# megvii-research/basedet

Hardware: AMD Instinct MI355X
Metric: images/sec training RetinaNet-R50-FPN 1333x800 (higher is better)
Workload: dtype bf16; 1 GPU; retinanet_r50_800x1344 train step (fwd+bwd+allreduce+SGD), DummyLoader boxes, random-init weights, inputs resident in HBM; per_gpu_batch=16, global_batch=16, parallelism=dp1

## Files before the change

### basedet_amd/_lib.py

```python
import ctypes as C
import os

import torch

_HERE = os.path.dirname(os.path.abspath(__file__))
LIB_PATH = os.environ.get("BASEDET_HIP_LIB") or os.path.join(_HERE, "lib", "libbasedet_hip.so")

BD_MAX_SEGS = 8
ABI_VERSION = 112
EPI_RELU, EPI_ADD_BEFORE, EPI_ADD_AFTER, EPI_MASK, EPI_SPARSE = 1, 2, 4, 8, 16


class BasedetHipError(RuntimeError):
    pass


class ConvDesc(C.Structure):
    _fields_ = [
        ("N", C.c_int32), ("Cin", C.c_int32), ("Cout", C.c_int32), ("R", C.c_int32), ("S", C.c_int32),
        ("stride", C.c_int32), ("pad", C.c_int32), ("nseg", C.c_int32),
        ("Hi", C.c_int32 * BD_MAX_SEGS), ("Wi", C.c_int32 * BD_MAX_SEGS),
        ("Ho", C.c_int32 * BD_MAX_SEGS), ("Wo", C.c_int32 * BD_MAX_SEGS),
        ("in_off", C.c_int32 * BD_MAX_SEGS), ("out_off", C.c_int32 * BD_MAX_SEGS),
        ("in_pix_per_img", C.c_int32), ("out_pix_per_img", C.c_int32),
        ("route", C.c_int32 * 4), ("sr_seed", C.c_uint32),
        ("gskip", C.c_int32), ("gskip_ws", C.c_void_p), ("gskip_ws_bytes", C.c_size_t),
        ("gskip_gmap", C.c_void_p), ("gskip_gmap_bytes", C.c_size_t), ("gskip_dxmap", C.c_void_p), ("gskip_dxmap_bytes", C.c_size_t),
        ("gskip_dx_clean", C.c_int32),
        ("fwd_map", C.c_void_p), ("fwd_map_bytes", C.c_size_t), ("fwd_clean", C.c_int32),
    ]


class PackDesc(C.Structure):
    _fields_ = [("w", C.c_void_p), ("row_scale", C.c_void_p), ("w_fwd", C.c_void_p), ("w_dgrad", C.c_void_p),
                ("Cout", C.c_int32), ("RS", C.c_int32), ("Cin", C.c_int32), ("block_start", C.c_int32)]


class ImageDesc(C.Structure):
    _fields_ = [("offset", C.c_int64), ("src_h", C.c_int32), ("src_w", C.c_int32), ("dst_h", C.c_int32), ("dst_w", C.c_int32),
                ("flip", C.c_int32), ("reserved_", C.c_int32 * 1)]


_P, _I, _L, _F, _Z = C.c_void_p, C.c_int, C.c_int64, C.c_float, C.c_size_t
_D = C.POINTER(ConvDesc)

SIGNATURES = {
    "bd_last_error_string": (C.c_char_p, []),
    "bd_version": (_I, []),
    "bd_conv_last_kernel": (C.c_char_p, []),
# ... 113 lines not shown
    "bd_rcnn_loss_fwd_bwd": (_I, [_P, _I, _I, _I, _P, _P, _I, _F, _P, _P, _P, _P]),
    "bd_det_scores": (_I, [_P, _I, _P, _I, _I, _L, _I, _P, _P]),
    "bd_det_select_workspace_bytes": (_Z, [_I, _I, _L, _I, _I]),
    "bd_det_select": (_I, [_P, _I, _P, _I, _I, _I, _L, _I, _I, _P, _P, _I, _F, _P, _P, _P, _P, _Z, _P]),
    "bd_rcnn_predict": (_I, [_P, _I, _I, _I, _P, _P, _I, _I, _P, _P, _P, _P, _P]),
    "bd_det_candidates": (_I, [_I, _P, _P, _P, _I, _I, _I, _P, _I, _P, _P, _L, _I, _I, _P, _P, _P, _L, _P, _P, _P, _P]),
    "bd_det_finalize": (_I, [_P, _P, _P, _P, _P, _I, _I, _I, _P, _I, _P, _P, _P, _P]),
    "bd_sgd_momentum_step": (_I, [_P, _P, _P, _L, _F, _F, _F, _F, _P]),
    "bd_ema_update": (_I, [_P, _P, _L, _F, _F, _P]),
    "bd_sgd_momentum_ema_step": (_I, [_P, _P, _P, _P, _L, _F, _F, _F, _F, _F, _F, _P]),
    "bd_swap_f32": (_I, [_P, _P, _L, _P]),
    "bd_adam_step": (_I, [_P, _P, _P, _P, _L] + [_F] * 10 + [_I, _P]),
    "bd_adam_ema_step": (_I, [_P, _P, _P, _P, _P, _L] + [_F] * 10 + [_I, _F, _F, _P]),
    "bd_sgd_nesterov_step": (_I, [_P, _P, _P, _L, _F, _F, _F, _F, _P]),
    "bd_sgd_nesterov_ema_step": (_I, [_P, _P, _P, _P, _L, _F, _F, _F, _F, _F, _F, _P]),
    "bd_clip_grad_value": (_I, [_P, _L, _F, _F, _F, _P]),
    "bd_clip_grad_norm_workspace_bytes": (_Z, []),
    "bd_clip_grad_norm": (_I, [_P, _L, _F, _F, _F, _P, _P, _Z, _P]),
    "bd_quantize_fp8": (_I, [_P, _L, _F, _P, _P]),
    "bd_weight_pack_fp8": (_I, [_P, _P, _I, _I, _I, _F, _P, _P, _P]),
    "bd_conv2d_fwd_fp8": (_I, [_D, _P, _P, _P, _P, _P, _P, _I, _P]),
    "bd_conv2d_fwd_fp8_ex": (_I, [_D, _P, _P, _P, _P, _P, _P, _P, _F, _I, _P]),
    "bd_quantize_bf8": (_I, [_P, _L, _F, _P, C.c_uint32, _P]),
    "bd_absmax_bf16": (_I, [_P, _L, _P, _P]),
    "bd_weight_pack_fp8_t": (_I, [_P, _P, _I, _I, _I, _F, _P, _P, _P]),
    "bd_conv2d_dgrad_fp8": (_I, [_D, _P, _P, _P, _P, _P, _P, _P, _F, _I, _P]),
    "bd_conv2d_wgrad_fp8_workspace_bytes": (_Z, [_D]),
    "bd_conv2d_wgrad_fp8": (_I, [_D, _P, _P, _F, _P, _P, _I, _P, _Z, _P]),
    "bd_conv1x1_fp8": (_I, [_D, _I, _P, _P, _P, _P, _P, _P, _P, _P, _P, _P, _F, _I, _P]),
    "bd_sigmoid_focal_loss_elem": (_I, [_P, _P, _L, _F, _F, _P, _P, _P, _P]),
# ... 75 lines not shown
```

### basedet_amd/build.py

```python
import hashlib
import os
import subprocess
import sys

HERE = os.path.dirname(os.path.abspath(__file__))
CSRC = os.path.join(HERE, "csrc")
OUT_DIR = os.path.join(HERE, "lib")
LIB = os.path.join(OUT_DIR, os.environ.get("BD_LIB_NAME", "libbasedet_hip.so"))
HIPCC = os.environ.get("HIPCC", "/opt/rocm/bin/hipcc")
ARCH = "gfx950"

SOURCES = {
    "image_ops.hip": [],
    "image_resize.hip": ["-ffp-contract=off"],
    "ema.hip": [],
    "optim.hip": ["-ffp-contract=off", "-fhip-fp32-correctly-rounded-divide-sqrt"],
    "h2d.hip": [],
    "conv_igemm.hip": [],
    "conv3x3.hip": [],
    "conv3x3_pp.hip": [],
    "gskip.hip": [],
    "conv3x3_pp128.hip": [],
    "conv1x1.hip": [],
    "conv1x1_ring.hip": [],
    "conv1x1_thin.hip": [],
    "bottleneck_fused.hip": [],
    "conv_fp8.hip": [],
    "conv3x3_pp8.hip": [],
    "conv_wgrad.hip": [],
    "conv_wgrad3x3.hip": [],
    "conv_wgrad3x3_ring.hip": [],
# ... 88 lines not shown
```

### basedet_amd/csrc/ema.hip

```cpp
#include "common.h"

namespace {

__global__ void ema_kernel(float* __restrict__ e, const float* __restrict__ w, long long n, float m, float one_minus_m) {
    for (long long i = (long long)blockIdx.x * blockDim.x + threadIdx.x; i * 4 < n; i += (long long)gridDim.x * blockDim.x) {
        const long long o = i * 4;
        if (o + 4 <= n) {
            f32x4_t ev = *reinterpret_cast<f32x4_t*>(e + o);
            const f32x4_t wv = *reinterpret_cast<const f32x4_t*>(w + o);
#pragma unroll
            for (int k = 0; k < 4; ++k) ev[k] = ema_elem(ev[k], wv[k], m, one_minus_m);
            *reinterpret_cast<f32x4_t*>(e + o) = ev;
        } else {
            for (long long k = o; k < n; ++k) e[k] = ema_elem(e[k], w[k], m, one_minus_m);
        }
    }
}

__global__ void sgd_ema_kernel(float* __restrict__ w, float* __restrict__ v, const float* __restrict__ g, float* __restrict__ e,
                               long long n, float lr, float momentum, float wd, float grad_scale, float m, float one_minus_m) {
    for (long long i = (long long)blockIdx.x * blockDim.x + threadIdx.x; i * 4 < n; i += (long long)gridDim.x * blockDim.x) {
        const long long o = i * 4;
        if (o + 4 <= n) {
            f32x4_t wv = *reinterpret_cast<f32x4_t*>(w + o);
            f32x4_t vv = *reinterpret_cast<f32x4_t*>(v + o);
            const f32x4_t gv = *reinterpret_cast<const f32x4_t*>(g + o);
            f32x4_t ev = *reinterpret_cast<f32x4_t*>(e + o);
#pragma unroll
            for (int k = 0; k < 4; ++k) {
                const float gg = gv[k] * grad_scale + wd * wv[k];
                vv[k] = momentum * vv[k] + gg;
                wv[k] -= lr * vv[k];
                ev[k] = ema_elem(ev[k], wv[k], m, one_minus_m);
            }
            *reinterpret_cast<f32x4_t*>(w + o) = wv;
            *reinterpret_cast<f32x4_t*>(v + o) = vv;
            *reinterpret_cast<f32x4_t*>(e + o) = ev;
        } else {
            for (long long k = o; k < n; ++k) {
                const float gg = g[k] * grad_scale + wd * w[k];
                v[k] = momentum * v[k] + gg;
                w[k] -= lr * v[k];
                e[k] = ema_elem(e[k], w[k], m, one_minus_m);
            }
        }
    }
}

__global__ void swap_kernel(float* __restrict__ a, float* __restrict__ b, long long n) {
    for (long long i = (long long)blockIdx.x * blockDim.x + threadIdx.x; i * 4 < n; i += (long long)gridDim.x * blockDim.x) {
        const long long o = i * 4;
        if (o + 4 <= n) {
            const f32x4_t av = *reinterpret_cast<const f32x4_t*>(a + o);
            const f32x4_t bv = *reinterpret_cast<const f32x4_t*>(b + o);
            *reinterpret_cast<f32x4_t*>(a + o) = bv;
            *reinterpret_cast<f32x4_t*>(b + o) = av;
        } else {
            for (long long k = o; k < n; ++k) {
// ... 48 lines not shown
```

### basedet_amd/csrc/image_ops.hip

```cpp
#include <stdarg.h>

#include <cmath>
#include "common.h"

static thread_local std::string g_bd_error = "";
int bd_num_cus() {
    static std::mutex mu;
    static int cached[256] = {0};
    int dev = 0;
    if (hipGetDevice(&dev) != hipSuccess || dev < 0 || dev > 255) return 256;
    std::lock_guard<std::mutex> g(mu);
    if (!cached[dev]) {
        int n = 0;
        cached[dev] = (hipDeviceGetAttribute(&n, hipDeviceAttributeMultiprocessorCount, dev) == hipSuccess && n > 0) ? n : 256;
    }
    return cached[dev];
}

void bd_set_error(const char* fmt, ...) {
    char buf[512];
    va_list ap;
    va_start(ap, fmt);
    vsnprintf(buf, sizeof(buf), fmt, ap);
    va_end(ap);
    g_bd_error = buf;
}
extern "C" const char* bd_last_error_string(void) { return g_bd_error.c_str(); }
static thread_local const char* g_bd_last_kernel = "";
void bd_note_kernel(const char* name) { g_bd_last_kernel = name; }
extern "C" const char* bd_conv_last_kernel(void) { return g_bd_last_kernel; }
extern "C" int bd_version(void) { return 112; }

namespace {

constexpr int HALO_Y = 3, HALO_X = 4;

__global__ void pad_normalize_kernel(const float* __restrict__ in, int N, int H, int W, int Hp, int Wp,
                                     float m0, float m1, float m2, float s0, float s1, float s2,
                                     bf16_raw* __restrict__ out) {
    const int Hb = Hp + 2 * HALO_Y, Wb = Wp + 2 * HALO_X;
    const long long total = (long long)N * Hb * Wb;
    for (long long i = (long long)blockIdx.x * blockDim.x + threadIdx.x; i < total; i += (long long)gridDim.x * blockDim.x) {
        const int xb = (int)(i % Wb);
        const long long t = i / Wb;
        const int yb = (int)(t % Hb);
        const int n = (int)(t / Hb);
// ... 295 lines not shown
        for (int k = 0; k < 32; ++k) t += red[k * 8 + cl];
        out[c] = accumulate ? out[c] + t : t;
    }
}

__global__ void sgd_kernel(float* __restrict__ w, float* __restrict__ v, const float* __restrict__ g, long long n,
                           float lr, float momentum, float wd, float grad_scale) {
    for (long long i = (long long)blockIdx.x * blockDim.x + threadIdx.x; i * 4 < n; i += (long long)gridDim.x * blockDim.x) {
        const long long e = i * 4;
        if (e + 4 <= n) {
            f32x4_t wv = *reinterpret_cast<f32x4_t*>(w + e);
            f32x4_t vv = *reinterpret_cast<f32x4_t*>(v + e);
            const f32x4_t gv = *reinterpret_cast<const f32x4_t*>(g + e);
#pragma unroll
            for (int k = 0; k < 4; ++k) {
                const float gg = gv[k] * grad_scale + wd * wv[k];
                vv[k] = momentum * vv[k] + gg;
                wv[k] -= lr * vv[k];
            }
            *reinterpret_cast<f32x4_t*>(w + e) = wv;
            *reinterpret_cast<f32x4_t*>(v + e) = vv;
        } else {
            for (long long k = e; k < n; ++k) {
                const float gg = g[k] * grad_scale + wd * w[k];
                v[k] = momentum * v[k] + gg;
                w[k] -= lr * v[k];
            }
        }
    }
}

}

extern "C" int bd_pad_normalize(const float* in, int N, int H, int W, int Hp, int Wp, const float* mean3,
                                const float* std3, void* out, bd_stream_t stream) {
    BD_REQUIRE(in && out && mean3 && std3, "pad_normalize: null pointer");
    BD_REQUIRE(Hp >= H && Wp >= W && N > 0, "pad_normalize: padded size smaller than input");
    const long long total = (long long)N * (Hp + 6) * (Wp + 8);
    hipLaunchKernelGGL(pad_normalize_kernel, dim3(grid_for(total)), dim3(256), 0, (hipStream_t)stream, in, N, H, W, Hp, Wp,
                       mean3[0], mean3[1], mean3[2], std3[0], std3[1], std3[2], (bf16_raw*)out);
    BD_CHECK_LAUNCH("bd_pad_normalize");
// ... 238 lines not shown
```

### basedet_amd/csrc/optim.hip

```cpp
#include "common.h"

namespace {

struct AdamArgs {
    float lr, beta1, one_minus_beta1, beta2, one_minus_beta2, bc1, bc2, eps, wd, grad_scale, ema_m, one_minus_ema_m;
};

template <bool DECOUPLED, bool EMA>
__device__ __forceinline__ void adam_elem(float& w, float& m, float& v, float g, float& e, const AdamArgs& a) {
    float gg = g * a.grad_scale;
    if (!DECOUPLED) gg = gg + a.wd * w;
    m = a.beta1 * m + a.one_minus_beta1 * gg;
    v = a.beta2 * v + a.one_minus_beta2 * (gg * gg);
    float d = (m / a.bc1) / (sqrtf(v / a.bc2) + a.eps);
    if (DECOUPLED) d = d + a.wd * w;
    w = w - a.lr * d;
    if (EMA) e = ema_elem(e, w, a.ema_m, a.one_minus_ema_m);
}

template <bool DECOUPLED, bool EMA>
__global__ void adam_kernel(float* __restrict__ w, float* __restrict__ m, float* __restrict__ v, const float* __restrict__ g,
                            float* __restrict__ e, long long n, AdamArgs a) {
    for (long long i = (long long)blockIdx.x * blockDim.x + threadIdx.x; i * 4 < n; i += (long long)gridDim.x * blockDim.x) {
        const long long o = i * 4;
        if (o + 4 <= n) {
            f32x4_t wv = *reinterpret_cast<f32x4_t*>(w + o);
            f32x4_t mv = *reinterpret_cast<f32x4_t*>(m + o);
            f32x4_t vv = *reinterpret_cast<f32x4_t*>(v + o);
            const f32x4_t gv = *reinterpret_cast<const f32x4_t*>(g + o);
            f32x4_t ev = {0.f, 0.f, 0.f, 0.f};
            if (EMA) ev = *reinterpret_cast<f32x4_t*>(e + o);
#pragma unroll
            for (int k = 0; k < 4; ++k) {
// ... 2 lines not shown
                wv[k] = wk; mv[k] = mk; vv[k] = vk; ev[k] = ek;
            }
            *reinterpret_cast<f32x4_t*>(w + o) = wv;
            *reinterpret_cast<f32x4_t*>(m + o) = mv;
            *reinterpret_cast<f32x4_t*>(v + o) = vv;
            if (EMA) *reinterpret_cast<f32x4_t*>(e + o) = ev;
        } else {
            for (long long k = o; k < n; ++k) {
                float wk = w[k], mk = m[k], vk = v[k], ek = EMA ? e[k] : 0.f;
                adam_elem<DECOUPLED, EMA>(wk, mk, vk, g[k], ek, a);
                w[k] = wk; m[k] = mk; v[k] = vk;
                if (EMA) e[k] = ek;
            }
        }
    }
}

template <bool EMA>
__device__ __forceinline__ void nesterov_elem(float& w, float& v, float g, float& e, float lr, float momentum, float wd, float grad_scale,
                                              float ema_m, float one_minus_ema_m) {
    const float gg = g * grad_scale + wd * w;
    v = momentum * v + gg;
    w -= lr * (gg + momentum * v);
    if (EMA) e = ema_elem(e, w, ema_m, one_minus_ema_m);
}

template <bool EMA>
__global__ void sgd_nesterov_kernel(float* __restrict__ w, float* __restrict__ v, const float* __restrict__ g, float* __restrict__ e,
                                    long long n, float lr, float momentum, float wd, float grad_scale, float ema_m,
                                    float one_minus_ema_m) {
    for (long long i = (long long)blockIdx.x * blockDim.x + threadIdx.x; i * 4 < n; i += (long long)gridDim.x * blockDim.x) {
        const long long o = i * 4;
        if (o + 4 <= n) {
            f32x4_t wv = *reinterpret_cast<f32x4_t*>(w + o);
            f32x4_t vv = *reinterpret_cast<f32x4_t*>(v + o);
            const f32x4_t gv = *reinterpret_cast<const f32x4_t*>(g + o);
            f32x4_t ev = {0.f, 0.f, 0.f, 0.f};
            if (EMA) ev = *reinterpret_cast<f32x4_t*>(e + o);
#pragma unroll
// ... 94 lines not shown
```

### basedet_amd/models/fpn_base.py

```python
import math

import numpy as np
import torch

from .. import ops
from ..data.raw import RawImageBatch
from ..ops import Geom
from ..streams import SideStreams, fork, join
from . import params as P
from .. import comm as _comm
from .engine import ConvLayer, DeconvLayer, FCLayer, ParamArena, TrainableStem
from .fp8_scaling import Fp8GradScaler, initial_grad_scale
from .live_norm import BatchNormState, LiveNorms
from .plan_arena import PlanArena, _Carver, _Plan, _round_up
from .wgrad_sched import WgradScheduler


class VecParam:

    def __init__(self, name, numel):
        self.name, self.numel = name, numel
        self.w = self.g = None

    def reserve(self, arena):
# ... 252 lines not shown
    def _q8_buf(self, key, nbytes):
        t = self._q8.get(key)
        if t is None or t.numel() < nbytes:
            t = self._q8[key] = torch.empty((int(nbytes),), dtype=torch.uint8, device=self.device)
        return t

    def load_weights(self, weights, strict=False):
        from ..utils.checkpoint import load_matched_weights
        return load_matched_weights(self, weights, strict)

    def repack_weights(self):
        ops.stem_weight_pack(self.stem_w, self.stem_scale, self.stem_packed)
        for c in self.convs.values():
            c.pack()

    def repack_trainable(self):
        self.fp8_scaler.apply_staged()
        if self._pack_table is None:
            ent = [(c.w, c.row_scale, c.w_fwd, c.w_dgrad, c.cout, c.k * c.k, c.cin) for c in self.convs.values()
                   if c.trainable and not isinstance(c, DeconvLayer)]
            self._pack_table = ops.build_pack_table(ent, self.device)
        ops.weight_pack_multi(self._pack_table)
        if self.stem is not None:
            ops.stem_weight_pack(self.stem_w, self.stem_scale, self.stem_packed)
        for c in self.upsample.values():
            c.pack()
        for c in self.convs.values():
            if (c.fp8 or c.fp8_1x1 or c.fp8_1x1_dgrad) and c.trainable:
                c.pack_fp8()
        if self.norms and not self.training:
            self._fold_norms()

    def _fold_norms(self, pack=True):
        if not self.norms:
            return
        for c in self.convs.values():
            if c.norm is None:
# ... 689 lines not shown
```

### basedet_amd/ops.py

```python
import ctypes as C
from dataclasses import dataclass, field
from typing import List, Optional

import torch

from . import _lib
from ._lib import ConvDesc, EPI_ADD_AFTER, EPI_ADD_BEFORE, EPI_MASK, EPI_RELU, EPI_SPARSE, check, f32arr, i32arr, ptr, stream_ptr


@dataclass
class Geom:
    N: int
    H: List[int]
    W: List[int]
    off: List[int] = field(default_factory=list)
    pix_per_img: int = 0

    def __post_init__(self):
        if not self.off:
            o = 0
            self.off = []
            for h, w in zip(self.H, self.W):
                self.off.append(o)
                o += h * w
# ... 295 lines not shown
        arr[i].w = w.data_ptr()
        arr[i].row_scale = rs.data_ptr() if rs is not None else None
        arr[i].w_fwd = wf.data_ptr() if wf is not None else None
        arr[i].w_dgrad = wd.data_ptr() if wd is not None else None
        arr[i].Cout, arr[i].RS, arr[i].Cin, arr[i].block_start = co, r, ci, start
        start += int(L().bd_weight_pack_blocks(co, r, ci))
    raw = np.frombuffer(bytes(arr), dtype=np.uint8).copy()
    return torch.from_numpy(raw).to(device), len(entries), start


def weight_pack_multi(table):
    t, n, blocks = table
    check(L().bd_weight_pack_multi(ptr(t), n, blocks, stream_ptr()), "bd_weight_pack_multi")


def colsum_workspace_bytes(Cn):
    return int(L().bd_colsum_workspace_bytes(Cn))


def colsum_bf16(g, rows, Cn, out, ws, accumulate=False, geom=None):
    if geom is None:
        n, ppi, off, cnt = 1, rows, 0, rows
    else:
        assert geom.nlev == 1
        n, ppi, off, cnt = geom.N, geom.pix_per_img, geom.off[0], geom.H[0] * geom.W[0]
    check(L().bd_colsum_bf16(ptr(g), n, ppi, off, cnt, Cn, ptr(out), int(accumulate), ptr(ws), ws.numel() * ws.element_size(),
                             stream_ptr()), "bd_colsum_bf16")
    return out


# ... 446 lines not shown
                                  stream_ptr()), "bd_fcos_offsets_fwd")
    return out


def fcos_offsets_workspace_bytes():
    return int(L().bd_fcos_offsets_workspace_bytes())


def fcos_offsets_bwd(raw, ld, scales, geom: Geom, strides, d_off, d_ctr, d_raw, dscale, ws):
    off, cnt = _lvl_arrays(geom)
    check(L().bd_fcos_offsets_bwd(ptr(raw), ld, ptr(scales), geom.N, geom.nlev, off, cnt, i32arr(strides), geom.pix_per_img, ptr(d_off),
                                  ptr(d_ctr), ptr(d_raw), ptr(dscale), ptr(ws), ws.numel() * ws.element_size(), stream_ptr()),
          "bd_fcos_offsets_bwd")


def sgd_momentum_step(w, v, g, lr, momentum, wd, grad_scale=1.0):
    check(L().bd_sgd_momentum_step(ptr(w), ptr(v), ptr(g), w.numel(), float(lr), float(momentum), float(wd),
                                   float(grad_scale), stream_ptr()), "bd_sgd_momentum_step")


def ema_coeffs(m):
    return float(m), float(1 - m)


def _same_f32(*ts):
    assert all(t.dtype == torch.float32 and t.numel() == ts[0].numel() for t in ts), "fp32 buffers of one length expected"


def ema_update(e, w, m):
    _same_f32(e, w)
    mm, om = ema_coeffs(m)
    check(L().bd_ema_update(ptr(e), ptr(w), e.numel(), mm, om, stream_ptr()), "bd_ema_update")


def sgd_momentum_ema_step(w, v, g, e, lr, momentum, wd, grad_scale, m):
    _same_f32(w, v, g, e)
    mm, om = ema_coeffs(m)
    check(L().bd_sgd_momentum_ema_step(ptr(w), ptr(v), ptr(g), ptr(e), w.numel(), float(lr), float(momentum), float(wd),
                                       float(grad_scale), mm, om, stream_ptr()), "bd_sgd_momentum_ema_step")


def swap_f32(a, b):
    _same_f32(a, b)
    check(L().bd_swap_f32(ptr(a), ptr(b), a.numel(), stream_ptr()), "bd_swap_f32")


def adam_coeffs(betas, step):
    b1, b2 = float(betas[0]), float(betas[1])
    return b1, 1 - b1, b2, 1 - b2, 1 - b1 ** step, 1 - b2 ** step


def adam_step(w, m, v, g, lr, betas, eps, wd, step, grad_scale=1.0, decoupled=False):
    _same_f32(w, m, v, g)
    check(L().bd_adam_step(ptr(w), ptr(m), ptr(v), ptr(g), w.numel(), float(lr), *adam_coeffs(betas, step), float(eps), float(wd),
                           float(grad_scale), int(bool(decoupled)), stream_ptr()), "bd_adam_step")


def adam_ema_step(w, m, v, g, e, lr, betas, eps, wd, step, grad_scale, decoupled, ema_m):
    _same_f32(w, m, v, g, e)
    mm, om = ema_coeffs(ema_m)
    check(L().bd_adam_ema_step(ptr(w), ptr(m), ptr(v), ptr(g), ptr(e), w.numel(), float(lr), *adam_coeffs(betas, step), float(eps),
                               float(wd), float(grad_scale), int(bool(decoupled)), mm, om, stream_ptr()), "bd_adam_ema_step")


def sgd_nesterov_step(w, v, g, lr, momentum, wd, grad_scale=1.0):
    _same_f32(w, v, g)
    check(L().bd_sgd_nesterov_step(ptr(w), ptr(v), ptr(g), w.numel(), float(lr), float(momentum), float(wd), float(grad_scale),
                                   stream_ptr()), "bd_sgd_nesterov_step")


def sgd_nesterov_ema_step(w, v, g, e, lr, momentum, wd, grad_scale, m):
    _same_f32(w, v, g, e)
    mm, om = ema_coeffs(m)
    check(L().bd_sgd_nesterov_ema_step(ptr(w), ptr(v), ptr(g), ptr(e), w.numel(), float(lr), float(momentum), float(wd),
                                       float(grad_scale), mm, om, stream_ptr()), "bd_sgd_nesterov_ema_step")


class WgradQueue:

    def __init__(self):
        self._h = C.c_void_p()
        check(L().bd_wgrad_queue_create(C.byref(self._h)), "bd_wgrad_queue_create")

    def wgrad(self, d, x, g, dw, dbias, ws, row_scale=None, accumulate=False):
        check(L().bd_conv2d_wgrad_queued(self._h, C.byref(_stamp(d)), ptr(x), ptr(g), ptr(row_scale), ptr(dw), ptr(dbias), int(accumulate), ptr(ws),
                                         ws.numel() * ws.element_size(), stream_ptr()), "bd_conv2d_wgrad_queued")
# ... 79 lines not shown
```

### basedet_amd/solver/__init__.py

```python
import torch

from .. import comm as _comm
from .. import ops
from ..streams import fork, join
from ..utils.registry import registers


class _ParamGroupView(dict):
    pass


def _moments_out(model, buf):
    w = model.arena.w
    ops.swap_f32(buf, w)
    try:
        states = model.state_dict()
    finally:
        ops.swap_f32(buf, w)
    return {k: states[k] for k in model.state_dict_trainable_names()}


def _moments_in(model, buf, values):
    own = model.state_dict()
    trainable = set(model.state_dict_trainable_names())
    missing = sorted(trainable - set(values))
    if missing:
        raise ValueError(f"optimizer state lacks {len(missing)} trainable parameter(s), e.g. {missing[0]!r}")
    merged = {k: (values[k] if k in trainable else v) for k, v in own.items()}
    w = model.arena.w
    try:
        ops.swap_f32(buf, w)
        try:
            model._bind_params(merged)
        finally:
            ops.swap_f32(buf, w)
    finally:
        model.repack_weights()


class SGD:

    def __init__(self, model, lr, weight_decay, momentum=0.9, nesterov=False):
        if nesterov and momentum <= 0:
            raise ValueError("SGD: nesterov=True requires a momentum > 0")
        self.model = model
        self.nesterov = bool(nesterov)
        self.step_count = 0
        self.param_groups = [_ParamGroupView(lr=lr, weight_decay=weight_decay, momentum=momentum)]

    def step(self, grad_scale=1.0, ema=None):
        a = self.model.arena
        g = self.param_groups[0]
        m = ema.fused_momentum() if ema is not None else None
        plain, fused = (ops.sgd_nesterov_step, ops.sgd_nesterov_ema_step) if self.nesterov else \
            (ops.sgd_momentum_step, ops.sgd_momentum_ema_step)
        if m is None:
            plain(a.w, a.v, a.g, g["lr"], g["momentum"], g["weight_decay"], grad_scale)
        else:
            fused(a.w, a.v, a.g, ema.e, g["lr"], g["momentum"], g["weight_decay"], grad_scale, m)
        self.step_count += 1
        self.model.repack_trainable()
        return self

    def clear_grad(self):
        return self

    def state_dict(self):
        return {"step": self.step_count, "momentum_buffer": _moments_out(self.model, self.model.arena.v)}

    def load_state_dict(self, states):
        self.step_count = int(states["step"])
        _moments_in(self.model, self.model.arena.v, states["momentum_buffer"])


class Adam:

    decoupled = False

    def __init__(self, model, lr, weight_decay, betas=(0.9, 0.999), eps=1e-8):
        if len(betas) != 2 or not all(0.0 <= float(b) < 1.0 for b in betas):
            raise ValueError(f"{type(self).__name__}: betas must be two values in [0, 1), got {betas!r}")
        betas = (float(betas[0]), float(betas[1]))
        if eps < 0:
            raise ValueError(f"{type(self).__name__}: eps must not be negative, got {eps!r}")
        self.model = model
        self.step_count = 0
        self.param_groups = [_ParamGroupView(lr=lr, weight_decay=weight_decay, betas=betas, eps=eps)]
        a = model.arena
        self.exp_avg_sq = torch.zeros(a.total, dtype=torch.float32, device=a.w.device)

    def step(self, grad_scale=1.0, ema=None):
        a = self.model.arena
        g = self.param_groups[0]
        m = ema.fused_momentum() if ema is not None else None
        t = self.step_count + 1
        if m is None:
            ops.adam_step(a.w, a.v, self.exp_avg_sq, a.g, g["lr"], g["betas"], g["eps"], g["weight_decay"], t, grad_scale,
                          self.decoupled)
        else:
            ops.adam_ema_step(a.w, a.v, self.exp_avg_sq, a.g, ema.e, g["lr"], g["betas"], g["eps"], g["weight_decay"], t, grad_scale,
                              self.decoupled, m)
        self.step_count = t
        self.model.repack_trainable()
        return self

    def clear_grad(self):
        return self

    def state_dict(self):
        return {"step": self.step_count, "exp_avg": _moments_out(self.model, self.model.arena.v),
                "exp_avg_sq": _moments_out(self.model, self.exp_avg_sq)}

    def load_state_dict(self, states):
        self.step_count = int(states["step"])
        _moments_in(self.model, self.model.arena.v, states["exp_avg"])
        _moments_in(self.model, self.exp_avg_sq, states["exp_avg_sq"])


# ... 187 lines not shown
class DetSolver:
    @classmethod
    def build(cls, cfg, model):
        solver_cfg = cfg.SOLVER
        mode = solver_cfg.get("REDUCE_MODE", "MEAN")
        assert mode in ["MEAN", "SUM"]
        world = _comm.world_size()
        lr = solver_cfg.BASIC_LR * cfg.MODEL.BATCHSIZE
        wd = solver_cfg.WEIGHT_DECAY
        if mode == "MEAN":
            lr = lr * world
        else:
            wd = wd * world
        extra = dict(solver_cfg.get("EXTRA_OPT_ARGS", {}))
        opt = build_optimizer(solver_cfg.get("OPTIMIZER_NAME", "SGD"), model, lr, wd, extra)
        amp = cfg.get("TRAINER", {}).get("AMP", {}) if hasattr(cfg, "get") else {}
        scaler = None
        if amp.get("ENABLE", False):
            dyn = bool(amp.get("DYNAMIC_SCALE", False))
            scaler = GradScaler(65536.0 if dyn else 128.0, 2000 if dyn else 0)
        return Solver(opt, GradBuckets(model, mode, wire_dtype=str(solver_cfg.get("ALLREDUCE_DTYPE", "fp32"))), grad_scaler=scaler)


def broadcast_parameters(model, src=0):
    c = _comm.get_comm()
    if c is not None and c.world > 1:
        c.bcast(model.arena.w, root=src)
        if getattr(model, "norms", None):
            c.bcast(model.norms.running, root=src)
        model.repack_trainable()
# ... 1 lines not shown
```

### include/basedet_hip.h

```cpp
#ifndef BASEDET_HIP_H
#define BASEDET_HIP_H

#include <stddef.h>
#include <stdint.h>

#ifdef __cplusplus
extern "C" {
#endif

#define BD_OK 0
#define BD_EINVAL (-1)
#define BD_ELAUNCH (-2)
#define BD_EWORKSPACE (-3)

#define BD_MAX_SEGS 8

#define BD_EPI_RELU 1
#define BD_EPI_ADD_BEFORE 2
#define BD_EPI_ADD_AFTER 4
#define BD_EPI_MASK 8
#define BD_EPI_SPARSE 16

typedef void* bd_stream_t;

// ... 356 lines not shown
int bd_ema_update(float* e, const float* w, int64_t n, float m, float one_minus_m, bd_stream_t stream);
int bd_sgd_momentum_ema_step(float* w, float* v, const float* g, float* e, int64_t n, float lr, float momentum, float wd,
                             float grad_scale, float m, float one_minus_m, bd_stream_t stream);
int bd_swap_f32(float* a, float* b, int64_t n, bd_stream_t stream);

int bd_adam_step(float* w, float* m, float* v, const float* g, int64_t n, float lr, float beta1, float one_minus_beta1, float beta2,
                 float one_minus_beta2, float bc1, float bc2, float eps, float wd, float grad_scale, int decoupled, bd_stream_t stream);
int bd_adam_ema_step(float* w, float* m, float* v, const float* g, float* e, int64_t n, float lr, float beta1, float one_minus_beta1,
                     float beta2, float one_minus_beta2, float bc1, float bc2, float eps, float wd, float grad_scale, int decoupled,
                     float ema_m, float one_minus_ema_m, bd_stream_t stream);
int bd_sgd_nesterov_step(float* w, float* v, const float* g, int64_t n, float lr, float momentum, float wd, float grad_scale,
                         bd_stream_t stream);
int bd_sgd_nesterov_ema_step(float* w, float* v, const float* g, float* e, int64_t n, float lr, float momentum, float wd,
                             float grad_scale, float ema_m, float one_minus_ema_m, bd_stream_t stream);

int bd_quantize_fp8(const void* x_bf16, int64_t n, float scale, void* q, bd_stream_t stream);
int bd_weight_pack_fp8(const float* w, const float* row_scale, int Cout, int RS, int Cin, float act_scale, void* wq, float* wscale,
                       bd_stream_t stream);
int bd_conv2d_fwd_fp8(const bd_conv_desc* d, const void* xq, const void* wq, const float* wscale, const float* bias, const void* add,
                      void* y, int flags, bd_stream_t stream);
int bd_conv2d_fwd_fp8_ex(const bd_conv_desc* d, const void* xq, const void* wq, const float* wscale, const float* bias, const void* add,
                         void* y, void* y8, float q_scale, int flags, bd_stream_t stream);
int bd_quantize_bf8(const void* x_bf16, int64_t n, float scale, void* q, uint32_t sr_seed, bd_stream_t stream);
int bd_absmax_bf16(const void* x_bf16, int64_t n, float* out, bd_stream_t stream);
int bd_weight_pack_fp8_t(const float* w, const float* row_scale, int Cout, int RS, int Cin, float grad_scale, void* wq_t, float* wscale_t,
                         bd_stream_t stream);
int bd_conv2d_dgrad_fp8(const bd_conv_desc* d, const void* g8, const void* wq_t, const float* wscale_t, const void* add, const void* mask,
                        void* dx, void* dx8, float q_scale, int flags, bd_stream_t stream);
size_t bd_conv1x1_thin_bwd_workspace_bytes(void);
int bd_conv1x1_thin_fwd(const void* x, const float* w, const float* bias, int64_t M, int Cin, int Cout, void* y, bd_stream_t stream);
// ... 54 lines not shown
```

Baseline: 723.6 images/sec.

## Fuse optimizer step with bf16 weight repacking in one table-driven kernel

```diff
diff --git a/basedet_amd/_lib.py b/basedet_amd/_lib.py
--- a/basedet_amd/_lib.py
+++ b/basedet_amd/_lib.py
@@ -7,7 +7,7 @@
 LIB_PATH = os.environ.get("BASEDET_HIP_LIB") or os.path.join(_HERE, "lib", "libbasedet_hip.so")
 
 BD_MAX_SEGS = 8
-ABI_VERSION = 112
+ABI_VERSION = 113
 EPI_RELU, EPI_ADD_BEFORE, EPI_ADD_AFTER, EPI_MASK, EPI_SPARSE = 1, 2, 4, 8, 16
 
 
@@ -33,6 +33,11 @@
 
 class PackDesc(C.Structure):
     _fields_ = [("w", C.c_void_p), ("row_scale", C.c_void_p), ("w_fwd", C.c_void_p), ("w_dgrad", C.c_void_p),
+                ("Cout", C.c_int32), ("RS", C.c_int32), ("Cin", C.c_int32), ("block_start", C.c_int32)]
+
+
+class StepDesc(C.Structure):
+    _fields_ = [("off", C.c_int64), ("count", C.c_int64), ("row_scale", C.c_void_p), ("w_fwd", C.c_void_p), ("w_dgrad", C.c_void_p),
                 ("Cout", C.c_int32), ("RS", C.c_int32), ("Cin", C.c_int32), ("block_start", C.c_int32)]
 
 
@@ -176,6 +181,8 @@
     "bd_adam_ema_step": (_I, [_P, _P, _P, _P, _P, _L] + [_F] * 10 + [_I, _F, _F, _P]),
     "bd_sgd_nesterov_step": (_I, [_P, _P, _P, _L, _F, _F, _F, _F, _P]),
     "bd_sgd_nesterov_ema_step": (_I, [_P, _P, _P, _P, _L, _F, _F, _F, _F, _F, _F, _P]),
+    "bd_optim_pack_blocks": (_I, [_I, _I, _L]),
+    "bd_optim_pack_step": (_I, [_I, _P, _I, _I, _P, _P, _P, _P, _P, _L] + [_F] * 13 + [_P]),
     "bd_clip_grad_value": (_I, [_P, _L, _F, _F, _F, _P]),
     "bd_clip_grad_norm_workspace_bytes": (_Z, []),
     "bd_clip_grad_norm": (_I, [_P, _L, _F, _F, _F, _P, _P, _Z, _P]),
diff --git a/basedet_amd/build.py b/basedet_amd/build.py
--- a/basedet_amd/build.py
+++ b/basedet_amd/build.py
@@ -15,6 +15,7 @@
     "image_resize.hip": ["-ffp-contract=off"],
     "ema.hip": [],
     "optim.hip": ["-ffp-contract=off", "-fhip-fp32-correctly-rounded-divide-sqrt"],
+    "optim_pack.hip": ["-fhip-fp32-correctly-rounded-divide-sqrt"],
     "h2d.hip": [],
     "conv_igemm.hip": [],
     "conv3x3.hip": [],
diff --git a/basedet_amd/csrc/ema.hip b/basedet_amd/csrc/ema.hip
--- a/basedet_amd/csrc/ema.hip
+++ b/basedet_amd/csrc/ema.hip
@@ -1,4 +1,5 @@
 #include "common.h"
+#include "optim_dev.h"
 
 namespace {
 
@@ -28,20 +29,20 @@
             f32x4_t ev = *reinterpret_cast<f32x4_t*>(e + o);
 #pragma unroll
             for (int k = 0; k < 4; ++k) {
-                const float gg = gv[k] * grad_scale + wd * wv[k];
-                vv[k] = momentum * vv[k] + gg;
-                wv[k] -= lr * vv[k];
-                ev[k] = ema_elem(ev[k], wv[k], m, one_minus_m);
+                float wk = wv[k], vk = vv[k];
+                sgd_elem(wk, vk, gv[k], lr, momentum, wd, grad_scale);
+                wv[k] = wk; vv[k] = vk;
+                ev[k] = ema_elem(ev[k], wk, m, one_minus_m);
             }
             *reinterpret_cast<f32x4_t*>(w + o) = wv;
             *reinterpret_cast<f32x4_t*>(v + o) = vv;
             *reinterpret_cast<f32x4_t*>(e + o) = ev;
         } else {
             for (long long k = o; k < n; ++k) {
-                const float gg = g[k] * grad_scale + wd * w[k];
-                v[k] = momentum * v[k] + gg;
-                w[k] -= lr * v[k];
-                e[k] = ema_elem(e[k], w[k], m, one_minus_m);
+                float wk = w[k], vk = v[k];
+                sgd_elem(wk, vk, g[k], lr, momentum, wd, grad_scale);
+                w[k] = wk; v[k] = vk;
+                e[k] = ema_elem(e[k], wk, m, one_minus_m);
             }
         }
     }
diff --git a/basedet_amd/csrc/image_ops.hip b/basedet_amd/csrc/image_ops.hip
--- a/basedet_amd/csrc/image_ops.hip
+++ b/basedet_amd/csrc/image_ops.hip
@@ -2,6 +2,7 @@
 
 #include <cmath>
 #include "common.h"
+#include "optim_dev.h"
 
 static thread_local std::string g_bd_error = "";
 int bd_num_cus() {
@@ -29,7 +30,7 @@
 static thread_local const char* g_bd_last_kernel = "";
 void bd_note_kernel(const char* name) { g_bd_last_kernel = name; }
 extern "C" const char* bd_conv_last_kernel(void) { return g_bd_last_kernel; }
-extern "C" int bd_version(void) { return 112; }
+extern "C" int bd_version(void) { return 113; }
 
 namespace {
 
@@ -355,17 +356,17 @@
             const f32x4_t gv = *reinterpret_cast<const f32x4_t*>(g + e);
 #pragma unroll
             for (int k = 0; k < 4; ++k) {
-                const float gg = gv[k] * grad_scale + wd * wv[k];
-                vv[k] = momentum * vv[k] + gg;
-                wv[k] -= lr * vv[k];
+                float wk = wv[k], vk = vv[k];
+                sgd_elem(wk, vk, gv[k], lr, momentum, wd, grad_scale);
+                wv[k] = wk; vv[k] = vk;
             }
             *reinterpret_cast<f32x4_t*>(w + e) = wv;
             *reinterpret_cast<f32x4_t*>(v + e) = vv;
         } else {
             for (long long k = e; k < n; ++k) {
-                const float gg = g[k] * grad_scale + wd * w[k];
-                v[k] = momentum * v[k] + gg;
-                w[k] -= lr * v[k];
+                float wk = w[k], vk = v[k];
+                sgd_elem(wk, vk, g[k], lr, momentum, wd, grad_scale);
+                w[k] = wk; v[k] = vk;
             }
         }
     }
diff --git a/basedet_amd/csrc/optim.hip b/basedet_amd/csrc/optim.hip
--- a/basedet_amd/csrc/optim.hip
+++ b/basedet_amd/csrc/optim.hip
@@ -1,22 +1,7 @@
 #include "common.h"
+#include "optim_dev.h"
 
 namespace {
-
-struct AdamArgs {
-    float lr, beta1, one_minus_beta1, beta2, one_minus_beta2, bc1, bc2, eps, wd, grad_scale, ema_m, one_minus_ema_m;
-};
-
-template <bool DECOUPLED, bool EMA>
-__device__ __forceinline__ void adam_elem(float& w, float& m, float& v, float g, float& e, const AdamArgs& a) {
-    float gg = g * a.grad_scale;
-    if (!DECOUPLED) gg = gg + a.wd * w;
-    m = a.beta1 * m + a.one_minus_beta1 * gg;
-    v = a.beta2 * v + a.one_minus_beta2 * (gg * gg);
-    float d = (m / a.bc1) / (sqrtf(v / a.bc2) + a.eps);
-    if (DECOUPLED) d = d + a.wd * w;
-    w = w - a.lr * d;
-    if (EMA) e = ema_elem(e, w, a.ema_m, a.one_minus_ema_m);
-}
 
 template <bool DECOUPLED, bool EMA>
 __global__ void adam_kernel(float* __restrict__ w, float* __restrict__ m, float* __restrict__ v, const float* __restrict__ g,
@@ -49,15 +34,6 @@
             }
         }
     }
-}
-
-template <bool EMA>
-__device__ __forceinline__ void nesterov_elem(float& w, float& v, float g, float& e, float lr, float momentum, float wd, float grad_scale,
-                                              float ema_m, float one_minus_ema_m) {
-    const float gg = g * grad_scale + wd * w;
-    v = momentum * v + gg;
-    w -= lr * (gg + momentum * v);
-    if (EMA) e = ema_elem(e, w, ema_m, one_minus_ema_m);
 }
 
 template <bool EMA>
diff --git a/basedet_amd/csrc/optim_dev.h b/basedet_amd/csrc/optim_dev.h
--- /dev/null
+++ b/basedet_amd/csrc/optim_dev.h
@@ -0,0 +1,36 @@
+#pragma once
+#include "common.h"
+
+struct AdamArgs {
+    float lr, beta1, one_minus_beta1, beta2, one_minus_beta2, bc1, bc2, eps, wd, grad_scale, ema_m, one_minus_ema_m;
+};
+
+__device__ __forceinline__ void sgd_elem(float& w, float& v, float g, float lr, float momentum, float wd, float grad_scale) {
+#pragma clang fp contract(off)
+    const float gg = __builtin_fmaf(g, grad_scale, wd * w);
+    v = __builtin_fmaf(momentum, v, gg);
+    w = __builtin_fmaf(-lr, v, w);
+}
+
+template <bool EMA>
+__device__ __forceinline__ void nesterov_elem(float& w, float& v, float g, float& e, float lr, float momentum, float wd, float grad_scale,
+                                              float ema_m, float one_minus_ema_m) {
+#pragma clang fp contract(off)
+    const float gg = g * grad_scale + wd * w;
+    v = momentum * v + gg;
+    w -= lr * (gg + momentum * v);
+    if (EMA) e = ema_elem(e, w, ema_m, one_minus_ema_m);
+}
+
+template <bool DECOUPLED, bool EMA>
+__device__ __forceinline__ void adam_elem(float& w, float& m, float& v, float g, float& e, const AdamArgs& a) {
+#pragma clang fp contract(off)
+    float gg = g * a.grad_scale;
+    if (!DECOUPLED) gg = gg + a.wd * w;
+    m = a.beta1 * m + a.one_minus_beta1 * gg;
+    v = a.beta2 * v + a.one_minus_beta2 * (gg * gg);
+    float d = (m / a.bc1) / (sqrtf(v / a.bc2) + a.eps);
+    if (DECOUPLED) d = d + a.wd * w;
+    w = w - a.lr * d;
+    if (EMA) e = ema_elem(e, w, a.ema_m, a.one_minus_ema_m);
+}
diff --git a/basedet_amd/csrc/optim_pack.hip b/basedet_amd/csrc/optim_pack.hip
--- /dev/null
+++ b/basedet_amd/csrc/optim_pack.hip
@@ -0,0 +1,161 @@
+#include "common.h"
+#include "optim_dev.h"
+
+namespace {
+
+template <int MODE, bool EMA>
+__device__ __forceinline__ void step_elem(float& w, float& v, float& s, float g, float& e, const AdamArgs& a, float momentum) {
+    if constexpr (MODE == BD_OPTIM_SGD) {
+        sgd_elem(w, v, g, a.lr, momentum, a.wd, a.grad_scale);
+        if (EMA) e = ema_elem(e, w, a.ema_m, a.one_minus_ema_m);
+    } else if constexpr (MODE == BD_OPTIM_NESTEROV) {
+        nesterov_elem<EMA>(w, v, g, e, a.lr, momentum, a.wd, a.grad_scale, a.ema_m, a.one_minus_ema_m);
+    } else {
+        adam_elem<MODE == BD_OPTIM_ADAMW, EMA>(w, v, s, g, e, a);
+    }
+}
+
+constexpr bool has_s(int mode) { return mode == BD_OPTIM_ADAM || mode == BD_OPTIM_ADAMW; }
+
+template <int MODE, bool EMA>
+__device__ __forceinline__ f32x4_t step4(long long o, float* __restrict__ w, float* __restrict__ v, float* __restrict__ s,
+                                         const float* __restrict__ g, float* __restrict__ e, const AdamArgs& a, float momentum) {
+    f32x4_t wv = *reinterpret_cast<f32x4_t*>(w + o);
+    f32x4_t vv = *reinterpret_cast<f32x4_t*>(v + o);
+    const f32x4_t gv = *reinterpret_cast<const f32x4_t*>(g + o);
+    f32x4_t sv = {0.f, 0.f, 0.f, 0.f}, ev = {0.f, 0.f, 0.f, 0.f};
+    if (has_s(MODE)) sv = *reinterpret_cast<f32x4_t*>(s + o);
+    if (EMA) ev = *reinterpret_cast<f32x4_t*>(e + o);
+#pragma unroll
+    for (int k = 0; k < 4; ++k) {
+        float wk = wv[k], vk = vv[k], sk = sv[k], ek = ev[k];
+        step_elem<MODE, EMA>(wk, vk, sk, gv[k], ek, a, momentum);
+        wv[k] = wk; vv[k] = vk; sv[k] = sk; ev[k] = ek;
+    }
+    *reinterpret_cast<f32x4_t*>(w + o) = wv;
+    *reinterpret_cast<f32x4_t*>(v + o) = vv;
+    if (has_s(MODE)) *reinterpret_cast<f32x4_t*>(s + o) = sv;
+    if (EMA) *reinterpret_cast<f32x4_t*>(e + o) = ev;
+    return wv;
+}
+
+constexpr int FLAT_PER_BLOCK = 1024;
+
+template <int MODE, bool EMA>
+__global__ __launch_bounds__(256) void optim_pack_kernel(const bd_step_desc* __restrict__ descs, int n, float* __restrict__ w,
+                                                         float* __restrict__ v, float* __restrict__ s, const float* __restrict__ g,
+                                                         float* __restrict__ e, AdamArgs a, float momentum) {
+    __shared__ float tile[32][33];
+    int lo = 0, hi = n - 1;
+    const int b = blockIdx.x;
+    while (lo < hi) {
+        const int mid = (lo + hi + 1) >> 1;
+        if (descs[mid].block_start <= b) lo = mid; else hi = mid - 1;
+    }
+    const bd_step_desc d = descs[lo];
+    int t = b - d.block_start;
+    if (d.RS == 0) {
+        const long long end = d.off + d.count;
+        const long long o = d.off + (long long)t * FLAT_PER_BLOCK + threadIdx.x * 4;
+        if (o + 4 <= end) {
+            step4<MODE, EMA>(o, w, v, s, g, e, a, momentum);
+        } else {
+            for (long long k = o; k < end; ++k) {
+                float wk = w[k], vk = v[k], sk = has_s(MODE) ? s[k] : 0.f, ek = EMA ? e[k] : 0.f;
+                step_elem<MODE, EMA>(wk, vk, sk, g[k], ek, a, momentum);
+                w[k] = wk; v[k] = vk;
+                if (has_s(MODE)) s[k] = sk;
+                if (EMA) e[k] = ek;
+            }
+        }
+        return;
+    }
+    const int ci_tiles = (d.Cin + 31) / 32, co_tiles = (d.Cout + 31) / 32;
+    const int ci_t = t % ci_tiles; t /= ci_tiles;
+    const int co_t = t % co_tiles;
+    const int tap = t / co_tiles;
+    bf16_raw* wf = (bf16_raw*)d.w_fwd;
+    bf16_raw* wd = (bf16_raw*)d.w_dgrad;
+    const int row = threadIdx.x >> 3, q = threadIdx.x & 7;
+    {
+        const int co = co_t * 32 + row, ci = ci_t * 32 + q * 4;
+        f32x4_t wv = {0.f, 0.f, 0.f, 0.f};
+        if (co < d.Cout && ci < d.Cin) {
+            const long long i = ((long long)co * d.RS + tap) * d.Cin + ci;
+            wv = step4<MODE, EMA>(d.off + i, w, v, s, g, e, a, momentum);
+            if (d.row_scale) {
+                const float rs = d.row_scale[co];
+#pragma unroll
+                for (int k = 0; k < 4; ++k) wv[k] *= rs;
+            }
+            if (wf) {
+                u32x2_t p;
+                p[0] = (uint32_t)f2bf(wv[0]) | ((uint32_t)f2bf(wv[1]) << 16);
+                p[1] = (uint32_t)f2bf(wv[2]) | ((uint32_t)f2bf(wv[3]) << 16);
+                *reinterpret_cast<u32x2_t*>(wf + i) = p;
+            }
+        }
+#pragma unroll
+        for (int k = 0; k < 4; ++k) tile[row][q * 4 + k] = wv[k];
+    }
+    __syncthreads();
+    if (wd) {
+        const int ci = ci_t * 32 + row, co = co_t * 32 + q * 4;
+        if (ci < d.Cin && co < d.Cout) {
+            u32x2_t p;
+            p[0] = (uint32_t)f2bf(tile[q * 4 + 0][row]) | ((uint32_t)f2bf(tile[q * 4 + 1][row]) << 16);
+            p[1] = (uint32_t)f2bf(tile[q * 4 + 2][row]) | ((uint32_t)f2bf(tile[q * 4 + 3][row]) << 16);
+            *reinterpret_cast<u32x2_t*>(wd + ((long long)ci * d.RS + tap) * d.Cout + co) = p;
+        }
+    }
+}
+
+inline bool aligned16(const void* p) { return ((uintptr_t)p & 15u) == 0; }
+inline bool disjoint(const float* a, const float* b, int64_t n) { return a + n <= b || b + n <= a; }
+
+template <int MODE>
+void launch(bool ema, int blocks, hipStream_t st, const bd_step_desc* descs, int n, float* w, float* v, float* s, const float* g, float* e,
+            const AdamArgs& a, float momentum) {
+    if (ema) hipLaunchKernelGGL((optim_pack_kernel<MODE, true>), dim3(blocks), dim3(256), 0, st, descs, n, w, v, s, g, e, a, momentum);
+    else hipLaunchKernelGGL((optim_pack_kernel<MODE, false>), dim3(blocks), dim3(256), 0, st, descs, n, w, v, s, g, e, a, momentum);
+}
+
+}
+
+extern "C" int bd_optim_pack_blocks(int Cout, int RS, int64_t Cin_or_count) {
+    if (RS == 0) return (int)((Cin_or_count + FLAT_PER_BLOCK - 1) / FLAT_PER_BLOCK);
+    return RS * ((Cout + 31) / 32) * (((int)Cin_or_count + 31) / 32);
+}
+
+extern "C" int bd_optim_pack_step(int mode, const bd_step_desc* descs_dev, int n, int total_blocks, float* w, float* v, float* s,
+                                  const float* g, float* e, int64_t total, float lr, float wd, float grad_scale, float momentum,
+                                  float beta1, float one_minus_beta1, float beta2, float one_minus_beta2, float bc1, float bc2, float eps,
+                                  float ema_m, float one_minus_ema_m, bd_stream_t stream) {
+    BD_REQUIRE(mode >= BD_OPTIM_SGD && mode <= BD_OPTIM_ADAMW, "optim_pack_step: unknown mode %d", mode);
+    BD_REQUIRE(descs_dev && n > 0 && total_blocks > 0 && total > 0, "optim_pack_step: bad arguments");
+    const bool adam = has_s(mode), ema = e != nullptr;
+    BD_REQUIRE(w && v && g && (s || !adam), "optim_pack_step: null pointer");
+    BD_REQUIRE(aligned16(w) && aligned16(v) && aligned16(g) && aligned16(e) && (!adam || aligned16(s)),
+               "optim_pack_step: every arena must be 16-byte aligned");
+    BD_REQUIRE(disjoint(v, w, total) && disjoint(g, w, total) && disjoint(g, v, total), "optim_pack_step: w, v and g overlap");
+    if (adam) {
+        BD_REQUIRE(disjoint(s, w, total) && disjoint(s, v, total) && disjoint(s, g, total), "optim_pack_step: s overlaps w, v or g");
+        BD_REQUIRE(beta1 >= 0.f && beta1 < 1.f && beta2 >= 0.f && beta2 < 1.f, "optim_pack_step: betas must lie in [0, 1)");
+        BD_REQUIRE(bc1 > 0.f && bc2 > 0.f, "optim_pack_step: bias corrections must be positive");
+        BD_REQUIRE(eps >= 0.f, "optim_pack_step: negative eps");
+    }
+    if (ema) {
+        BD_REQUIRE(disjoint(e, w, total) && disjoint(e, v, total) && disjoint(e, g, total) && (!adam || disjoint(e, s, total)),
+                   "optim_pack_step: e overlaps another arena");
+    }
+    const AdamArgs a = {lr, beta1, one_minus_beta1, beta2, one_minus_beta2, bc1, bc2, eps, wd, grad_scale, ema_m, one_minus_ema_m};
+    const hipStream_t st = (hipStream_t)stream;
+    switch (mode) {
+        case BD_OPTIM_SGD: launch<BD_OPTIM_SGD>(ema, total_blocks, st, descs_dev, n, w, v, s, g, e, a, momentum); break;
+        case BD_OPTIM_NESTEROV: launch<BD_OPTIM_NESTEROV>(ema, total_blocks, st, descs_dev, n, w, v, s, g, e, a, momentum); break;
+        case BD_OPTIM_ADAM: launch<BD_OPTIM_ADAM>(ema, total_blocks, st, descs_dev, n, w, v, s, g, e, a, momentum); break;
+        default: launch<BD_OPTIM_ADAMW>(ema, total_blocks, st, descs_dev, n, w, v, s, g, e, a, momentum); break;
+    }
+    BD_CHECK_LAUNCH("bd_optim_pack_step");
+    return BD_OK;
+}
diff --git a/basedet_amd/models/fpn_base.py b/basedet_amd/models/fpn_base.py
--- a/basedet_amd/models/fpn_base.py
+++ b/basedet_amd/models/fpn_base.py
@@ -290,13 +290,28 @@
         for c in self.convs.values():
             c.pack()
 
-    def repack_trainable(self):
+    def _pack_tables(self):
+        if self._pack_table is None:
+            convs = [c for c in self.convs.values() if c.trainable and not isinstance(c, DeconvLayer)]
+            ent = [(c.w, c.row_scale, c.w_fwd, c.w_dgrad, c.cout, c.k * c.k, c.cin) for c in convs]
+            base = self.arena.w.data_ptr()
+            off = [(c.w.data_ptr() - base) // 4 for c in convs]
+            tiled = [0 <= o <= self.arena.total - c.w.numel() and ops.step_tileable(o, c.cout, c.cin) for o, c in zip(off, convs)]
+            step = ops.build_step_table([(o,) + e[1:] for o, e, t in zip(off, ent, tiled) if t], self.arena.total, self.device)
+            rest = [e for e, t in zip(ent, tiled) if not t]
+            self._pack_table = (ops.build_pack_table(ent, self.device), step, ops.build_pack_table(rest, self.device) if rest else None)
+        return self._pack_table
+
+    def step_table(self):
+        return self._pack_tables()[1]
+
+    def repack_trainable(self, packed=False):
         self.fp8_scaler.apply_staged()
-        if self._pack_table is None:
-            ent = [(c.w, c.row_scale, c.w_fwd, c.w_dgrad, c.cout, c.k * c.k, c.cin) for c in self.convs.values()
-                   if c.trainable and not isinstance(c, DeconvLayer)]
-            self._pack_table = ops.build_pack_table(ent, self.device)
-        ops.weight_pack_multi(self._pack_table)
+        full, _, rest = self._pack_tables()
+        if not packed:
+            ops.weight_pack_multi(full)
+        elif rest is not None:
+            ops.weight_pack_multi(rest)
         if self.stem is not None:
             ops.stem_weight_pack(self.stem_w, self.stem_scale, self.stem_packed)
         for c in self.upsample.values():
diff --git a/basedet_amd/ops.py b/basedet_amd/ops.py
--- a/basedet_amd/ops.py
+++ b/basedet_amd/ops.py
@@ -333,6 +333,50 @@
     check(L().bd_weight_pack_multi(ptr(t), n, blocks, stream_ptr()), "bd_weight_pack_multi")
 
 
+OPTIM_SGD, OPTIM_NESTEROV, OPTIM_ADAM, OPTIM_ADAMW = 0, 1, 2, 3
+
+
+def step_tileable(off, Cout, Cin):
+    return off % 4 == 0 and Cout % 4 == 0 and Cin % 4 == 0
+
+
+def build_step_table(entries, total, device):
+    import numpy as np
+    from ._lib import StepDesc
+    rows, pos = [], 0
+    for off, rs, wf, wd, co, r, ci in sorted(entries, key=lambda t: t[0]):
+        assert off >= pos and step_tileable(off, co, ci) and r > 0, (off, pos, co, r, ci)
+        if off > pos:
+            rows.append((pos, off - pos, None, None, None, 0, 0, 0))
+        rows.append((off, co * r * ci, rs, wf, wd, co, r, ci))
+        pos = off + co * r * ci
+    assert pos <= total, (pos, total)
+    if pos < total:
+        rows.append((pos, total - pos, None, None, None, 0, 0, 0))
+    arr = (StepDesc * len(rows))()
+    start = 0
+    for i, (off, cnt, rs, wf, wd, co, r, ci) in enumerate(rows):
+        arr[i].off, arr[i].count = off, cnt
+        arr[i].row_scale = rs.data_ptr() if rs is not None else None
+        arr[i].w_fwd = wf.data_ptr() if wf is not None else None
+        arr[i].w_dgrad = wd.data_ptr() if wd is not None else None
+        arr[i].Cout, arr[i].RS, arr[i].Cin, arr[i].block_start = co, r, ci, start
+        start += int(L().bd_optim_pack_blocks(co, r, ci if r else cnt))
+    raw = np.frombuffer(bytes(arr), dtype=np.uint8).copy()
+    return torch.from_numpy(raw).to(device), len(rows), start
+
+
+def optim_pack_step(table, mode, w, v, s, g, e, lr, wd, grad_scale=1.0, momentum=0.0, betas=(0.0, 0.0), eps=0.0, step=1, ema_m=None):
+    t, n, blocks = table
+    adam = mode in (OPTIM_ADAM, OPTIM_ADAMW)
+    _same_f32(w, v, g, *([s] if adam else []), *([e] if ema_m is not None else []))
+    mm, om = ema_coeffs(ema_m) if ema_m is not None else (0.0, 0.0)
+    coeffs = adam_coeffs(betas, step) if adam else (0.0,) * 6
+    check(L().bd_optim_pack_step(int(mode), ptr(t), n, blocks, ptr(w), ptr(v), ptr(s) if adam else None, ptr(g),
+                                 ptr(e) if ema_m is not None else None, w.numel(), float(lr), float(wd), float(grad_scale), float(momentum),
+                                 *coeffs, float(eps), mm, om, stream_ptr()), "bd_optim_pack_step")
+
+
 def colsum_workspace_bytes(Cn):
     return int(L().bd_colsum_workspace_bytes(Cn))
 
@@ -809,7 +853,9 @@
           "bd_fcos_offsets_bwd")
 
 
-def sgd_momentum_step(w, v, g, lr, momentum, wd, grad_scale=1.0):
+def sgd_momentum_step(w, v, g, lr, momentum, wd, grad_scale=1.0, table=None):
+    if table is not None:
+        return optim_pack_step(table, OPTIM_SGD, w, v, None, g, None, lr, wd, grad_scale, momentum=momentum)
     check(L().bd_sgd_momentum_step(ptr(w), ptr(v), ptr(g), w.numel(), float(lr), float(momentum), float(wd),
                                    float(grad_scale), stream_ptr()), "bd_sgd_momentum_step")
 
@@ -828,7 +874,9 @@
     check(L().bd_ema_update(ptr(e), ptr(w), e.numel(), mm, om, stream_ptr()), "bd_ema_update")
 
 
-def sgd_momentum_ema_step(w, v, g, e, lr, momentum, wd, grad_scale, m):
+def sgd_momentum_ema_step(w, v, g, e, lr, momentum, wd, grad_scale, m, table=None):
+    if table is not None:
+        return optim_pack_step(table, OPTIM_SGD, w, v, None, g, e, lr, wd, grad_scale, momentum=momentum, ema_m=m)
     _same_f32(w, v, g, e)
     mm, om = ema_coeffs(m)
     check(L().bd_sgd_momentum_ema_step(ptr(w), ptr(v), ptr(g), ptr(e), w.numel(), float(lr), float(momentum), float(wd),
@@ -845,26 +893,36 @@
     return b1, 1 - b1, b2, 1 - b2, 1 - b1 ** step, 1 - b2 ** step
 
 
-def adam_step(w, m, v, g, lr, betas, eps, wd, step, grad_scale=1.0, decoupled=False):
+def adam_step(w, m, v, g, lr, betas, eps, wd, step, grad_scale=1.0, decoupled=False, table=None):
+    if table is not None:
+        return optim_pack_step(table, OPTIM_ADAMW if decoupled else OPTIM_ADAM, w, m, v, g, None, lr, wd, grad_scale, betas=betas, eps=eps,
+                               step=step)
     _same_f32(w, m, v, g)
     check(L().bd_adam_step(ptr(w), ptr(m), ptr(v), ptr(g), w.numel(), float(lr), *adam_coeffs(betas, step), float(eps), float(wd),
                            float(grad_scale), int(bool(decoupled)), stream_ptr()), "bd_adam_step")
 
 
-def adam_ema_step(w, m, v, g, e, lr, betas, eps, wd, step, grad_scale, decoupled, ema_m):
+def adam_ema_step(w, m, v, g, e, lr, betas, eps, wd, step, grad_scale, decoupled, ema_m, table=None):
+    if table is not None:
+        return optim_pack_step(table, OPTIM_ADAMW if decoupled else OPTIM_ADAM, w, m, v, g, e, lr, wd, grad_scale, betas=betas, eps=eps,
+                               step=step, ema_m=ema_m)
     _same_f32(w, m, v, g, e)
     mm, om = ema_coeffs(ema_m)
     check(L().bd_adam_ema_step(ptr(w), ptr(m), ptr(v), ptr(g), ptr(e), w.numel(), float(lr), *adam_coeffs(betas, step), float(eps),
                                float(wd), float(grad_scale), int(bool(decoupled)), mm, om, stream_ptr()), "bd_adam_ema_step")
 
 
-def sgd_nesterov_step(w, v, g, lr, momentum, wd, grad_scale=1.0):
+def sgd_nesterov_step(w, v, g, lr, momentum, wd, grad_scale=1.0, table=None):
+    if table is not None:
+        return optim_pack_step(table, OPTIM_NESTEROV, w, v, None, g, None, lr, wd, grad_scale, momentum=momentum)
     _same_f32(w, v, g)
     check(L().bd_sgd_nesterov_step(ptr(w), ptr(v), ptr(g), w.numel(), float(lr), float(momentum), float(wd), float(grad_scale),
                                    stream_ptr()), "bd_sgd_nesterov_step")
 
 
-def sgd_nesterov_ema_step(w, v, g, e, lr, momentum, wd, grad_scale, m):
+def sgd_nesterov_ema_step(w, v, g, e, lr, momentum, wd, grad_scale, m, table=None):
+    if table is not None:
+        return optim_pack_step(table, OPTIM_NESTEROV, w, v, None, g, e, lr, wd, grad_scale, momentum=momentum, ema_m=m)
     _same_f32(w, v, g, e)
     mm, om = ema_coeffs(m)
     check(L().bd_sgd_nesterov_ema_step(ptr(w), ptr(v), ptr(g), ptr(e), w.numel(), float(lr), float(momentum), float(wd),
diff --git a/basedet_amd/solver/__init__.py b/basedet_amd/solver/__init__.py
--- a/basedet_amd/solver/__init__.py
+++ b/basedet_amd/solver/__init__.py
@@ -38,12 +38,24 @@
         model.repack_weights()
 
 
+def _step_table(opt):
+    table = getattr(opt.model, "step_table", None)
+    if not opt.fused_pack or table is None or not opt.model.arena.w.is_cuda:
+        return {}
+    return {"table": table()}
+
+
+def _packed(table):
+    return {"packed": True} if table else {}
+
+
 class SGD:
 
     def __init__(self, model, lr, weight_decay, momentum=0.9, nesterov=False):
         if nesterov and momentum <= 0:
             raise ValueError("SGD: nesterov=True requires a momentum > 0")
         self.model = model
+        self.fused_pack = True
         self.nesterov = bool(nesterov)
         self.step_count = 0
         self.param_groups = [_ParamGroupView(lr=lr, weight_decay=weight_decay, momentum=momentum)]
@@ -52,14 +64,15 @@
         a = self.model.arena
         g = self.param_groups[0]
         m = ema.fused_momentum() if ema is not None else None
+        table = _step_table(self)
         plain, fused = (ops.sgd_nesterov_step, ops.sgd_nesterov_ema_step) if self.nesterov else \
             (ops.sgd_momentum_step, ops.sgd_momentum_ema_step)
         if m is None:
-            plain(a.w, a.v, a.g, g["lr"], g["momentum"], g["weight_decay"], grad_scale)
-        else:
-            fused(a.w, a.v, a.g, ema.e, g["lr"], g["momentum"], g["weight_decay"], grad_scale, m)
+            plain(a.w, a.v, a.g, g["lr"], g["momentum"], g["weight_decay"], grad_scale, **table)
+        else:
+            fused(a.w, a.v, a.g, ema.e, g["lr"], g["momentum"], g["weight_decay"], grad_scale, m, **table)
         self.step_count += 1
-        self.model.repack_trainable()
+        self.model.repack_trainable(**_packed(table))
         return self
 
     def clear_grad(self):
@@ -84,6 +97,7 @@
         if eps < 0:
             raise ValueError(f"{type(self).__name__}: eps must not be negative, got {eps!r}")
         self.model = model
+        self.fused_pack = True
         self.step_count = 0
         self.param_groups = [_ParamGroupView(lr=lr, weight_decay=weight_decay, betas=betas, eps=eps)]
         a = model.arena
@@ -94,14 +108,15 @@
         g = self.param_groups[0]
         m = ema.fused_momentum() if ema is not None else None
         t = self.step_count + 1
+        table = _step_table(self)
         if m is None:
             ops.adam_step(a.w, a.v, self.exp_avg_sq, a.g, g["lr"], g["betas"], g["eps"], g["weight_decay"], t, grad_scale,
-                          self.decoupled)
+                          self.decoupled, **table)
         else:
             ops.adam_ema_step(a.w, a.v, self.exp_avg_sq, a.g, ema.e, g["lr"], g["betas"], g["eps"], g["weight_decay"], t, grad_scale,
-                              self.decoupled, m)
+                              self.decoupled, m, **table)
         self.step_count = t
-        self.model.repack_trainable()
+        self.model.repack_trainable(**_packed(table))
         return self
 
     def clear_grad(self):
@@ -319,6 +334,7 @@
             wd = wd * world
         extra = dict(solver_cfg.get("EXTRA_OPT_ARGS", {}))
         opt = build_optimizer(solver_cfg.get("OPTIMIZER_NAME", "SGD"), model, lr, wd, extra)
+        opt.fused_pack = bool(solver_cfg.get("FUSED_PACK", True))
         amp = cfg.get("TRAINER", {}).get("AMP", {}) if hasattr(cfg, "get") else {}
         scaler = None
         if amp.get("ENABLE", False):
diff --git a/include/basedet_hip.h b/include/basedet_hip.h
--- a/include/basedet_hip.h
+++ b/include/basedet_hip.h
@@ -394,6 +394,20 @@
 int bd_sgd_nesterov_ema_step(float* w, float* v, const float* g, float* e, int64_t n, float lr, float momentum, float wd,
                              float grad_scale, float ema_m, float one_minus_ema_m, bd_stream_t stream);
 
+enum { BD_OPTIM_SGD = 0, BD_OPTIM_NESTEROV = 1, BD_OPTIM_ADAM = 2, BD_OPTIM_ADAMW = 3 };
+typedef struct bd_step_desc {
+    int64_t off, count;
+    const float* row_scale;
+    void* w_fwd;
+    void* w_dgrad;
+    int32_t Cout, RS, Cin, block_start;
+} bd_step_desc;
+int bd_optim_pack_blocks(int Cout, int RS, int64_t Cin_or_count);
+int bd_optim_pack_step(int mode, const bd_step_desc* descs_dev, int n, int total_blocks, float* w, float* v, float* s, const float* g,
+                       float* e, int64_t total, float lr, float wd, float grad_scale, float momentum, float beta1, float one_minus_beta1,
+                       float beta2, float one_minus_beta2, float bc1, float bc2, float eps, float ema_m, float one_minus_ema_m,
+                       bd_stream_t stream);
+
 int bd_quantize_fp8(const void* x_bf16, int64_t n, float scale, void* q, bd_stream_t stream);
 int bd_weight_pack_fp8(const float* w, const float* row_scale, int Cout, int RS, int Cin, float act_scale, void* wq, float* wscale,
                        bd_stream_t stream);
```

Measured after the change: 725.0 images/sec, median of 6. About the same (+0.2%).
